# Aster32/GAN-DANet

Measured on AMD Instinct MI355X. Metric: train samples/sec (G+D step) on 256x256 tiles, higher is better.
Workload: dtype bf16; 1 GPU; full G+D train step, 8ch 256x256 -> 1024x1024 tiles, batch 32/GPU (global 32), perceptual=on, SSIM evaluated, AdamW x2; survey_config=3, per_gpu_batch=32, global_batch=32, tile=256, parallelism=dp1

## Files before the change

gan-danet_amd/_lib.py:

```python
from __future__ import annotations

import ctypes as C
import os

HERE = os.path.dirname(os.path.abspath(__file__))
LIB_PATH = os.path.join(HERE, "lib", "libgandanet_hip.so")

PREC_FP32, PREC_BF16, PREC_X3 = 0, 1, 2
PAM_BWD_K64_ATOMIC, PAM_BWD_K64_PARTS, PAM_BWD_K32_PARTS, PAM_BWD_TWO_KERNEL = 0, 1, 2, 3
ACT_NONE, ACT_RELU, ACT_LEAKY02, ACT_SIGMOID = 0, 1, 2, 3
EVAL_F64, EVAL_SKIP_NAN = 1, 2
GUARD_SQNORM, GUARD_NORM, GUARD_COEF, GUARD_OK, GUARD_APPLIED, GUARD_SKIPPED, GUARD_RECORD = range(7)
GUARD_CHUNK = 65536
FILTER_F32, FILTER_F64 = 0, 1
EDGE_REFLECT, EDGE_INTERIOR = 0, 1
FILTER_MAX_RADIUS, SAVGOL_MAX_WINDOW = 64, 33
ZOOM_MIRROR, ZOOM_NEAREST = 0, 1
FREQ_MAX_BINS, FREQ_MAX_TABLE_BYTES = 33, 16 << 20
ZONE_MAX, ZONE_EDGE_CHUNK = 32, 512
STL_MAX_T = 2048

c_fp = C.c_void_p


# ... 151 lines not shown
    "gd_spline_prefilter_axis": (_i, [_p, _p, _i, _l, _l, _l, _p]),
    "gd_restore_units": (_i, [_p, _i, _p, _i, _p, _l, _l, C.c_double, C.c_double, C.c_double, _p, _i, _p]),
    "gd_masked_plane_mean_f64_ws_bytes": (_sz, [_l, _l]),
    "gd_masked_plane_mean_f64": (_i, [_p, _l, _l, _p, _p, _p, _p, _sz, _p]),
    "gd_blend_region": (_i, [_p, _p, _p, _i, _i, _i, _i, _i, _i, _i, _p]),
    "gd_channel_moments_ws_bytes": (_sz, [_l, _l]),
    "gd_channel_moments": (_i, [_p, _i, _l, _l, _p, _p, _sz, _p]),
    "gd_scale_from_moments_host": (_i, [C.POINTER(C.c_double), _l, C.POINTER(C.c_double), C.POINTER(C.c_double),
                                        C.POINTER(C.c_double)]),
    "gd_channel_affine": (_i, [_p, _i, _p, _i, _l, _l, _p, _p, _i, _l, _l, _p]),
    "gd_freq_cos_table_host": (_i, [_l, _i, C.POINTER(C.c_double)]),
    "gd_freq_augment_axis": (_i, [_p, _p, _i, _l, _l, _l, _p, _i, _p, _p]),
    "gd_zone_rasterize": (_i, [_p, _l, C.POINTER(_l), _i, _p, _l, _p, _l, _p, _p]),
    "gd_zone_rasterize_host": (_i, [C.POINTER(C.c_double), _l, C.POINTER(_l), _i, C.POINTER(C.c_double), _l, C.POINTER(C.c_double), _l,
                                    C.POINTER(C.c_uint32)]),
    "gd_zone_mean_ws_bytes": (_sz, [_l, _l, _i]),
    "gd_zone_mean": (_i, [_p, _i, _l, _l, _p, _i, _p, _p, _p, _p, _sz, _p]),
    "gd_stl_decompose": (_i, [_p, _i, _l, _l, _i, _i, _i, _i, _i, _i, _i, _i, _i, _p, _p, _p, _p, _p]),
    "gd_stl_decompose_host": (_i, [_p, _i, _l, _l, _i, _i, _i, _i, _i, _i, _i, _i, _i, _p, _p, _p, _p]),
    "gd_augment_d4": (_i, [_p, _p, _i, _i, _i, _i, _p, _p, _f, _p]),
    "gd_bcast_mul": (_i, [_p, _p, _p, _i, _i, _l, _i, _p]),
    "gd_row_dot": (_i, [_p, _p, _p, _l, _l, _p]),
    "gd_chan_maxmean_fwd": (_i, [_p, _p, _p, _i, _i, _l, _p]),
    "gd_chan_maxmean_bwd": (_i, [_p, _p, _p, _i, _i, _l, _p]),
    "gd_comm_unique_id": (_i, [C.c_char_p]),
    "gd_comm_init": (_i, [_i, _i, C.c_char_p]),
    "gd_comm_world": (_i, []),
    "gd_allreduce": (_i, [_p, _sz, _i, _p]),
    "gd_reduce_scatter": (_i, [_p, _p, _sz, _i, _p]),
    "gd_allgather": (_i, [_p, _p, _sz, _i, _p]),
    "gd_comm_destroy": (_i, []),
    "gd_pack_bf16": (_i, [_p, _l, _i, _i, _i, _p, _f, _p, _i, _i, _p, _i, _i, _i, _i, _p]),
    "gd_pack_16": (_i, [_p, _l, _i, _i, _i, _p, _f, _p, _i, _i, _p, _i, _i, _i, _i, _i, _p]),
    "gd_pack_16_affine": (_i, [_p, _l, _i, _i, _i, _p, _p, _i, _p, _i, _i, _p, _i, _i, _i, _p]),
}

_lib = None


class GandanetError(RuntimeError):
    pass


def load() -> C.CDLL:
    global _lib
    if _lib is not None:
        return _lib
    if not os.path.exists(LIB_PATH):
        raise GandanetError(
            f"{LIB_PATH} is missing: the HIP extension is not built (run __graft_entry__.build()). "
            "There is no CPU fallback.")
    lib = C.CDLL(LIB_PATH)
    for name, (res, args) in SIGNATURES.items():
        fn = getattr(lib, name)
        fn.restype = res
        fn.argtypes = args
    if lib.gd_sizeof_conv_desc() != C.sizeof(ConvDesc) or lib.gd_sizeof_gemm_nt_desc() != C.sizeof(GemmNTDesc):
        raise GandanetError("descriptor struct layout differs between _lib.py and libgandanet_hip.so")
    _lib = lib
    return lib


def last_error() -> str:
    buf = C.create_string_buffer(512)
    load().gd_last_error(buf, 512)
    return buf.value.decode()
# ... 6 lines not shown
```

gan-danet_amd/csrc/gemm_conv.hip:

```cpp
#include <stdlib.h>

#include <type_traits>

#include "common.h"
#include "tile_mma.h"
#include "../../include/gandanet.h"

namespace {

using gd::TILE_BK;
using gd::TILE_BN;
constexpr int BN = TILE_BN;
constexpr int BK = TILE_BK;

template <int BM, int MODE>
__global__ __launch_bounds__(256) void conv_nn_kernel(const gd_conv_desc d) {
    constexpr bool BF16 = MODE != gd::MODE_F32;
    constexpr bool X3 = MODE == gd::MODE_X3;
    using P = gd::TilePol<MODE>;
    using elem = typename P::elem;
    constexpr int LD = P::LD;
    constexpr int WAVES_N = gd::TileGeom<BM>::WAVES_N;
    constexpr int TM = gd::TileGeom<BM>::TM;
    constexpr int TN = gd::TileGeom<BM>::TN;
// ... 450 lines not shown
    const float alpha = d.alpha ? *d.alpha : 1.f;
#pragma unroll
    for (int sb = 0; sb < NS; ++sb)
#pragma unroll
    for (int i = 0; i < TM; ++i)
#pragma unroll
        for (int j = 0; j < TN; ++j) {
            const int pn = n0 + sb * BN + wn * TN * 32 + j * 32 + r;
            if (pn >= HW) continue;
            float rsv[16], oldv[16];
#pragma unroll
            for (int e = 0; e < 16; ++e) {
                const int m = m0 + wm * TM * 32 + i * 32 + gd::acc_row(e, h);
                rsv[e] = (d.res && m < d.M) ? d.res[(long)b * d.res_bs + (long)m * HW + pn] : 0.f;
            }
#pragma unroll
            for (int e = 0; e < 16; ++e) {
                const int m = m0 + wm * TM * 32 + i * 32 + gd::acc_row(e, h);
                oldv[e] = (d.accumulate && m < d.M) ? reinterpret_cast<const float*>(d.y)[(long)b * d.y_bs + (long)m * HW + pn] : 0.f;
            }
#pragma unroll
            for (int e = 0; e < 16; ++e) {
                const int m = m0 + wm * TM * 32 + i * 32 + gd::acc_row(e, h);
                if (m >= d.M) continue;
                float v = acc[sb][i][j][e] * alpha + rsv[e];
                if (d.bias) v += d.bias[m];
                if (d.act == GD_ACT_RELU) v = fmaxf(v, 0.f);
                else if (d.act == GD_ACT_LEAKY02) v = v >= 0.f ? v : 0.2f * v;
                reinterpret_cast<float*>(d.y)[(long)b * d.y_bs + (long)m * HW + pn] = v + oldv[e];
            }
        }
}

template <int BM, bool X3 = false>
__global__ __launch_bounds__(256) void conv1x1_tr_plain_kernel(const gd_conv_desc d) {
    constexpr int LDA = BK + 8;
    constexpr int A_PL = BM * LDA, X_PL = BK * XLD;
    constexpr int WAVES_N = gd::TileGeom<BM>::WAVES_N;
    constexpr int TM = gd::TileGeom<BM>::TM;
    constexpr int TN = gd::TileGeom<BM>::TN;
    constexpr int KPT_A = BM / 8;
    __shared__ __attribute__((aligned(16))) unsigned short As[(X3 ? 2 : 1) * BM * LDA];
    __shared__ __attribute__((aligned(16))) unsigned short Xs[(X3 ? 2 : 1) * BK * XLD];

    const int tid = threadIdx.x, lane = tid & 63, wave = tid >> 6;
    const int r = lane & 31, h = lane >> 5;
    const int wm = wave / WAVES_N, wn = wave % WAVES_N;
    const int b = blockIdx.z, m0 = blockIdx.y * BM, n0 = blockIdx.x * BN;
    const int HW = d.Ho * d.Wo;

    const int am = tid % BM, akg = tid / BM;
    const bool a_row_ok = (m0 + am) < d.M;
    const float* a_row = d.a + (long)b * d.a_bs + (long)(m0 + am) * d.a_sm;

    const int xq = tid & 31, xr0 = tid >> 5;
    const float* x_img = d.x + (long)b * d.x_bs;
    const int pq = n0 + xq * 4;
    const bool q_full = pq + 3 < HW;

    f32x16_t acc[TM][TN];
#pragma unroll
    for (int i = 0; i < TM; ++i)
#pragma unroll
        for (int j = 0; j < TN; ++j)
#pragma unroll
            for (int e = 0; e < 16; ++e) acc[i][j][e] = 0.f;

    float ra[KPT_A];
    float4 rx[4];
    const int T = (d.Ck + BK - 1) / BK;
    auto load_tile = [&](int t) {
        const int c0 = t * BK;
#pragma unroll
        for (int i = 0; i < KPT_A; ++i) {
            const int c = c0 + akg * KPT_A + i;
            ra[i] = (a_row_ok && c < d.Ck) ? a_row[(long)c * d.a_sc] : 0.f;
        }
#pragma unroll
        for (int i = 0; i < 4; ++i) {
            const int c = c0 + xr0 + 8 * i;
            float4 v = make_float4(0.f, 0.f, 0.f, 0.f);
            if (c < d.Ck) {
                const float* p = x_img + (long)c * HW + pq;
                if (q_full) {
                    v = *reinterpret_cast<const float4*>(p);
                } else {
// ... 104 lines not shown
            for (int i = 0; i < TM; ++i)
                fa[i] = *reinterpret_cast<const bf16x8_t*>(As + (wm * TM * 32 + i * 32 + r) * LDA + ks * 16 + 8 * h);
#pragma unroll
            for (int j = 0; j < TN; ++j) {
                const unsigned short* p = Xs + (ks * 16 + 8 * h + tq) * XLD + (wn * TN + j) * 32 + 16 * tg + 4 * tp;
                const s16x4_t lo = __builtin_amdgcn_ds_read_tr16_b64_v4i16((__attribute__((address_space(3))) s16x4_t*)p);
                const s16x4_t hi = __builtin_amdgcn_ds_read_tr16_b64_v4i16(
                    (__attribute__((address_space(3))) s16x4_t*)(p + 4 * XLD));
                fb[j] = bf16x8_t{lo.x, lo.y, lo.z, lo.w, hi.x, hi.y, hi.z, hi.w};
            }
#pragma unroll
            for (int i = 0; i < TM; ++i)
#pragma unroll
                for (int j = 0; j < TN; ++j)
                    acc[i][j] = __builtin_amdgcn_mfma_f32_32x32x16_bf16(
                        __builtin_bit_cast(gd::bf16x8_native_t, fa[i]), __builtin_bit_cast(gd::bf16x8_native_t, fb[j]),
                        acc[i][j], 0, 0, 0);
        }
    };

    load_tile(0);
    store_tile();
    __syncthreads();
    for (int t = 0; t < T; ++t) {
        if (t + 1 < T) load_tile(t + 1);
        compute_tile();
        __syncthreads();
        if (t + 1 < T) {
            store_tile();
            __syncthreads();
        }
    }

    const float alpha = d.alpha ? *d.alpha : 1.f;
#pragma unroll
    for (int i = 0; i < TM; ++i)
#pragma unroll
        for (int j = 0; j < TN; ++j) {
            const int pn = n0 + wn * TN * 32 + j * 32 + r;
            if (pn >= HW) continue;
            float rsv[16], oldv[16];
#pragma unroll
            for (int e = 0; e < 16; ++e) {
                const int m = m0 + wm * TM * 32 + i * 32 + gd::acc_row(e, h);
                rsv[e] = (d.res && m < d.M) ? d.res[(long)b * d.res_bs + (long)m * HW + pn] : 0.f;
            }
#pragma unroll
            for (int e = 0; e < 16; ++e) {
                const int m = m0 + wm * TM * 32 + i * 32 + gd::acc_row(e, h);
                oldv[e] = (d.accumulate && m < d.M) ? reinterpret_cast<const float*>(d.y)[(long)b * d.y_bs + (long)m * HW + pn] : 0.f;
            }
#pragma unroll
            for (int e = 0; e < 16; ++e) {
                const int m = m0 + wm * TM * 32 + i * 32 + gd::acc_row(e, h);
                if (m >= d.M) continue;
                float v = acc[i][j][e] * alpha + rsv[e];
                if (d.bias) v += d.bias[m];
                if (d.act == GD_ACT_RELU) v = fmaxf(v, 0.f);
                else if (d.act == GD_ACT_LEAKY02) v = v >= 0.f ? v : 0.2f * v;
                reinterpret_cast<float*>(d.y)[(long)b * d.y_bs + (long)m * HW + pn] = v + oldv[e];
            }
        }
}

static bool conv1x1_tr_eligible(const gd_conv_desc& d) {
    const long HW = (long)d.Ho * d.Wo;
    return d.ks == 1 && d.stride == 1 && d.pad == 0 && (d.precision == GD_PREC_BF16 || d.precision == GD_PREC_X3) && d.out_layout == 0 && !d.out_bf16 &&
           (d.Mstore == 0 || d.Mstore == d.M) && d.Hi == d.Ho && d.Wi == d.Wo && HW % 4 == 0 && d.x_bs % 4 == 0 &&
           ((uintptr_t)d.x % 16) == 0;
}

template <int BM>
int launch(const gd_conv_desc& d, hipStream_t s) {
    const int sstep = d.sub_step > 1 ? d.sub_step : 1;
    const long hs = (d.Ho - d.sub_oy + sstep - 1) / sstep, ws = (d.Wo - d.sub_ox + sstep - 1) / sstep;
    if (hs <= 0 || ws <= 0) return 0;
    dim3 grid(gd_cdiv(hs * ws, BN), gd_cdiv(d.Mstore, BM), d.B);
    if (d.precision == GD_PREC_BF16)
        hipLaunchKernelGGL((conv_nn_kernel<BM, gd::MODE_BF16>), grid, dim3(256), 0, s, d);
    else if (d.precision == GD_PREC_X3)
        hipLaunchKernelGGL((conv_nn_kernel<BM, gd::MODE_X3>), grid, dim3(256), 0, s, d);
    else
        hipLaunchKernelGGL((conv_nn_kernel<BM, gd::MODE_F32>), grid, dim3(256), 0, s, d);
    GD_LAUNCH_CHECK();
    return 0;
}

}

extern "C" int gd_conv2d(const gd_conv_desc* dp, void* stream) {
    GD_CHECK_ARG(dp != nullptr, "gd_conv2d: null descriptor");
    gd_conv_desc d = *dp;
    if (d.Mstore < d.M) d.Mstore = d.M;
    GD_CHECK_ARG(d.B > 0 && d.M > 0 && d.Ck > 0 && d.ks > 0 && d.stride > 0 && d.pad >= 0, "gd_conv2d: bad sizes");
    GD_CHECK_ARG(d.Hi > 0 && d.Wi > 0 && d.Ho > 0 && d.Wo > 0, "gd_conv2d: bad spatial sizes");
// ... 26 lines not shown
        if (d.precision == GD_PREC_X3) {
            if (bm == 32) hipLaunchKernelGGL((conv1x1_tr_plain_kernel<32, true>), grid, dim3(256), 0, s, d);
            else if (bm == 64) hipLaunchKernelGGL((conv1x1_tr_plain_kernel<64, true>), grid, dim3(256), 0, s, d);
            else hipLaunchKernelGGL((conv1x1_tr_plain_kernel<128, true>), grid, dim3(256), 0, s, d);
        } else if (ns == 1) {
            if (bm == 32) hipLaunchKernelGGL((conv1x1_tr_plain_kernel<32>), grid, dim3(256), 0, s, d);
            else if (bm == 64) hipLaunchKernelGGL((conv1x1_tr_plain_kernel<64>), grid, dim3(256), 0, s, d);
            else hipLaunchKernelGGL((conv1x1_tr_plain_kernel<128>), grid, dim3(256), 0, s, d);
        } else
        if (bm == 32) { if (ns == 4) GD_C1X1(32, 4); else if (ns == 2) GD_C1X1(32, 2); else GD_C1X1(32, 1); }
        else if (bm == 64) { if (ns == 4) GD_C1X1(64, 4); else if (ns == 2) GD_C1X1(64, 2); else GD_C1X1(64, 1); }
        else { if (ns == 2) GD_C1X1(128, 2); else GD_C1X1(128, 1); }
#undef GD_C1X1
        GD_LAUNCH_CHECK();
        return 0;
    }
    auto run = [&](const gd_conv_desc& dd) -> int {
        if (dd.Mstore <= 32) return launch<32>(dd, s);
        if (dd.Mstore <= 64 || (dd.Mstore % 128 != 0 && dd.Mstore % 128 <= 64)) return launch<64>(dd, s);
        return launch<128>(dd, s);
    };
    if (d.transposed && d.stride > 1 && d.sub_step <= 1) {
        for (int py = 0; py < d.stride; ++py)
            for (int px = 0; px < d.stride; ++px) {
                gd_conv_desc dd = d;
                dd.sub_oy = py; dd.sub_ox = px; dd.sub_step = d.stride;
                const int rc = run(dd);
                if (rc) return rc;
            }
        return 0;
    }
    return run(d);
}
```

gan-danet_amd/kern.py:

```python
from __future__ import annotations

import ctypes as C
import math
import os
from typing import Optional, Tuple

import torch

from . import _lib as L

Tensor = torch.Tensor


def _stream() -> int:
    return torch.cuda.current_stream().cuda_stream


def _ptr(t: Optional[Tensor]):
    return None if t is None else t.data_ptr()


def _chk(t: Tensor, name: str = "tensor", dtype=torch.float32) -> None:
    if not t.is_cuda:
        raise L.GandanetError(f"{name}: expected a GPU tensor (there is no CPU fallback in the product path)")
# ... 601 lines not shown
    db = torch.empty_like(b) if need_b else None
    L.check(lib().gd_ssim_bwd(_ptr(a), _ptr(b), _ptr(gscale), B, Cn, H, W, window, _ptr(coef), _ptr(da), _ptr(db),
                              _stream()), "gd_ssim_bwd")
    return da, db


def adamw(p: Tensor, g: Tensor, m: Tensor, v: Tensor, step: int, lr: float, beta1: float, beta2: float, eps: float,
          weight_decay: float, grad_scale: float = 1.0) -> None:
    for t in (p, g, m, v):
        _dense(t, "adamw tensor")
    L.check(lib().gd_adamw(_ptr(p), _ptr(g), _ptr(m), _ptr(v), p.numel(), step, lr, beta1, beta2, eps, weight_decay,
                           grad_scale, _stream()), "gd_adamw")


LOG2E = 1.4426950408889634


def pack_bf16(s: Tensor, R: int, Cc: int, *, scale: Optional[Tensor] = None, scale_imm: float = 1.0, plain_shape=None,
              t_shape=None, perm16: bool = False, ones_row: int = -1, f16: bool = False):
    sbs = _bview(s, "pack input")
    B = s.shape[0]
    plain = tr = None
    rp = ldp = ccp = ldt = 0
    dt = torch.float16 if f16 else torch.bfloat16
    if plain_shape is not None:
        rp, ldp = plain_shape
        plain = torch.empty(B, rp, ldp, device=s.device, dtype=dt)
    if t_shape is not None:
        ccp, ldt = t_shape
        tr = torch.empty(B, ccp, ldt, device=s.device, dtype=dt)
    L.check(lib().gd_pack_16(_ptr(s), sbs, B, R, Cc, _ptr(scale), float(scale_imm), _ptr(plain), rp, ldp, _ptr(tr),
                             ccp, ldt, int(perm16), int(ones_row), int(f16), _stream()), "gd_pack_16")
    return plain, tr


def pack_nhwc16_affine(x: Tensor, scale: Optional[Tensor], shift: Optional[Tensor], relu: bool) -> Tensor:
    sbs = _bview(x, "pack input")
    B, Cn, H, W = x.shape
    out = torch.empty(B, H * W, Cn, device=x.device, dtype=torch.bfloat16)
    L.check(lib().gd_pack_16_affine(_ptr(x), sbs, B, Cn, H * W, _ptr(scale), _ptr(shift), int(relu), None, 0, 0, _ptr(out),
                                    H * W, Cn, 0, _stream()), "gd_pack_16_affine")
    return out


def augment_d4(x: Tensor, ops: Tensor, noise: Optional[Tensor] = None, noise_scale: float = 0.05) -> Tensor:
    _dense(x, "augment input")
    _chk(ops, "augment ops", torch.int32)
    B, Cn, H, W = x.shape
    if ops.numel() != B or (noise is not None and _dense(noise, "noise").shape != x.shape):
        raise L.GandanetError("augment_d4: ops must hold one word per sample and noise must match the batch")
    y = torch.empty_like(x)
    L.check(lib().gd_augment_d4(_ptr(x), _ptr(y), B, Cn, H, W, _ptr(ops), _ptr(noise), float(noise_scale), _stream()),
            "gd_augment_d4")
    return y


def bcast_mul(x: Tensor, att: Tensor, mode: int) -> Tensor:
    _dense(x), _dense(att)
    B, Cn = x.shape[0], x.shape[1]
    HW = x[0, 0].numel()
    if att.numel() != (B * Cn if mode == 0 else B * HW):
        raise L.GandanetError(f"bcast_mul: gate of {att.numel()} elements does not match x {tuple(x.shape)} (mode {mode})")
    y = torch.empty_like(x)
    L.check(lib().gd_bcast_mul(_ptr(x), _ptr(att), _ptr(y), B, Cn, HW, mode, _stream()), "gd_bcast_mul")
    return y

# ... 962 lines not shown
```

gan-danet_amd/ops.py:

```python
from __future__ import annotations

import os
from typing import List, Optional

import torch
from torch.autograd import Function

from . import _lib as L
from . import kern as K
from .config import config, operand_mode, sixteen_bit

ACT_NONE, ACT_RELU, ACT_LEAKY, ACT_SIGMOID = L.ACT_NONE, L.ACT_RELU, L.ACT_LEAKY02, L.ACT_SIGMOID


def _prec(layer: str = "other") -> int:
    mode = operand_mode(layer)
    return L.PREC_BF16 if mode == "16" else L.PREC_X3 if mode == "x3" else L.PREC_FP32


def _x3(layer: str) -> bool:
    return operand_mode(layer) == "x3"


def _x3_eligible(x, w, stride, pad, act) -> bool:
# ... 32 lines not shown
        for w, b in zip(ws[1:], bs[1:]):
            acts.append(K.conv3x3_nhwc_s2(acts[-1], K.conv3x3_operator(_c(w), "fwd", sp), b, w.shape[0], 2, Disc1TrunkFn.SLOPE,
                                          split=sp))
        ctx.save_for_backward(x, *ws, *acts)
        ctx.has_bias = tuple(b is not None for b in bs)
        ctx.split = sp
        return K.nhwc_flatten_fwd(acts[-1], split=sp)

    @staticmethod
    def backward(ctx, df):
        x, *rest = ctx.saved_tensors
        ws, acts = rest[:4], rest[4:]
        need = ctx.needs_input_grad
        sp = ctx.split
        grads = [None] * 9
        g = K.nhwc_flatten_bwd(_c(df), acts[3], Disc1TrunkFn.SLOPE, split=sp)
        for l in (3, 2, 1):
            if need[1 + 2 * l] or need[2 + 2 * l]:
                dw, db = K.conv3x3_wgrad_nhwc(g, acts[l - 1], 2, ctx.has_bias[l] and need[2 + 2 * l], split=sp)
                grads[1 + 2 * l], grads[2 + 2 * l] = (dw if need[1 + 2 * l] else None), db
            g = K.conv3x3_nhwc_s2_dgrad(g, K.conv3x3_operator(_c(ws[l]), "dgrad_s2", sp), acts[l - 1], Disc1TrunkFn.SLOPE,
                                        split=sp)
        if need[1] or need[2]:
            dw, db = K.disc_stem_wgrad(g, x, ctx.has_bias[0] and need[2], split=sp)
            grads[1], grads[2] = (dw if need[1] else None), db
        if need[0]:
            grads[0] = K.disc_stem_dgrad(g, _c(ws[0]), x.shape[2], x.shape[3], split=sp)
        return tuple(grads)


CONV_WIDE_NHWC = os.environ.get("GD_CONV_WIDE_NHWC", "1") != "0"
DENSE_NHWC = os.environ.get("GD_DENSE_NHWC", "1") != "0"
PAM_CAT = os.environ.get("GD_PAM_CAT", "1") != "0"
WIDE_MIN_CIN = int(os.environ.get("GD_WIDE_MIN_CIN", "128"))


def _wide3x3(x, w, stride, pad, act, prec) -> bool:
    return (CONV_WIDE_NHWC and prec == L.PREC_BF16 and x.dim() == 4 and tuple(w.shape[2:]) == (3, 3) and stride == 1
            and pad == 1 and act in (ACT_NONE, ACT_RELU) and w.shape[1] >= WIDE_MIN_CIN and w.shape[1] % 8 == 0 and w.shape[0] > 32
            and w.shape[0] % 8 == 0 and (x.shape[2] * x.shape[3]) % 8 == 0)


def _pack3x3_x(x, split, scale=None, shift=None, relu=False):
    if split:
        return K.pack_split(x, scale=scale, shift=shift, relu=relu)[1]
    if scale is not None:
        return K.pack_nhwc16_affine(x, scale, shift, relu)
    B, Cin, H, W = x.shape
    return K.pack_bf16(x, Cin, H * W, t_shape=(H * W, Cin))[1]


def _packed3x3_fwd(x16, w, bias, H, W, split, relu=False, out=None):
    return K.conv3x3_nhwc_f32out(x16, K.conv3x3_operator(_c(w), "fwd", split), bias, w.shape[0], H, W, relu=relu, out=out)


def _packed3x3_bwd(dy, x16, w, H, W, split, need_dx, need_dw, mask=None, dw_first=False):
    if not (need_dx or need_dw):
        return None, None
    Cout, N = dy.shape[1], H * W
    if split:
        dyp, dyt = K.pack_split(_as3(dy), want_plain=need_dw, want_tr=need_dx, mask=None if mask is None else _as3(mask))
    else:
        dyp, dyt = K.pack_bf16(_as3(dy), Cout, N, plain_shape=(Cout, N) if need_dw else None,
                               t_shape=(N, Cout) if need_dx else None)

    def wgrad():
# ... 244 lines not shown


def _pad_plane(t: torch.Tensor, N: int, Np: int) -> torch.Tensor:
    if N == Np:
        return t
    B, R = t.shape[0], t.shape[1]
    out = torch.zeros(B, R, Np, device=t.device, dtype=torch.float32)
    K.copy_rows(t, K._bview(t), N, out, R * Np, Np, B, R, N)
    return out


def _pam_pack16(q, k, v, r, Cn, N, D, ones_row, f16):
    Np, Cp = _npad(N), _cp(Cn)
    _, qt = K.pack_bf16(q, r, N, scale_imm=K.LOG2E, t_shape=(Np, D), f16=f16)
    kn, kt = K.pack_bf16(k, r, N, plain_shape=(D, Np), t_shape=(Np, D), perm16=True, ones_row=D - 1, f16=f16)
    vn, vt = K.pack_bf16(v, Cn, N, plain_shape=(Cp, Np), t_shape=(Np, Cp), perm16=True, ones_row=ones_row, f16=f16)
    return qt, kt, kn, vn, vt


def _pam_route(B: int, Cn: int, r: int, N: int) -> str:
    if sixteen_bit("pam") and Cn <= 192 and r <= 31:
        return "narrow"
    if _pam_wide(Cn, r):
        return "wide"
    return "f32" if _pam_f32(B, Cn, r, N) else "chain"


def _pam_forward(x, wq, bq, wk, bk, wv, bv, gamma_p, out3, prec):
    B, Cn, H, W = x.shape
    N = H * W
    r = wq.shape[0]
    x3 = x.view(B, Cn, N)
    route = _pam_route(B, Cn, r, N)
    if route != "chain" and PAM_CAT and (bq is None) == (bk is None) == (bv is None):
        wc = torch.empty(2 * r + Cn, Cn, 1, 1, device=x.device, dtype=torch.float32)
        for w_, lo in ((wq, 0), (wk, r), (wv, 2 * r)):
            K.copy_slab(_c(w_).view(1, w_.shape[0], Cn), wc.view(1, 2 * r + Cn, Cn)[:, lo:lo + w_.shape[0]])
        bc = None
        if bq is not None:
            bc = torch.empty(2 * r + Cn, device=x.device, dtype=torch.float32)
            for b_, lo in ((bq, 0), (bk, r), (bv, 2 * r)):
                K.copy_slab(b_.view(1, -1, 1), bc.view(1, -1, 1)[:, lo:lo + b_.numel()])
        y3 = K.conv2d_fwd(x, wc, bc, 1, 0, prec).view(B, 2 * r + Cn, N)
        q, k, v = y3[:, :r], y3[:, r:2 * r], y3[:, 2 * r:]
    else:
        q = K.conv2d_fwd(x, wq, bq, 1, 0, prec).view(B, r, N)
        k = K.conv2d_fwd(x, wk, bk, 1, 0, prec).view(B, r, N)
        v = K.conv2d_fwd(x, wv, bv, 1, 0, prec).view(B, Cn, N)
    if route in ("narrow", "wide"):
        Np, Cp = _npad(N), _cp(Cn)
        f16 = _pam_f16()
        D = 32 if route == "narrow" else K.pam_wide_slots(r)
        ones = Cp - 1 if route == "narrow" and Cn < Cp else -1
        qt, kt, kn, vn, vt = _pam_pack16(q, k, v, r, Cn, N, D, ones, f16)
        del q, k, v
        y3 = None
        o_attn = torch.empty(B, Cn, N, device=x.device, dtype=torch.float32)
        lse = torch.empty(B, N, device=x.device, dtype=torch.float32)
        if route == "wide":
            K.pam_wide_fwd(qt, kt, vn, B, N, Np, Cn, Cp, D, gamma_p, x3, out3, o_attn, lse, r_alg=r, f16=f16)
        elif K.PAM_SHIFT and not f16:
            K.pam_flash_fwd_shift(qt, kt, vn, B, N, Np, Cn, Cp, gamma_p, x3, out3, o_attn, lse, r_alg=r, v_ones=ones >= 0)
        else:
            k_sqmax = K.pam_key_sqnorm_max(kt, N, f16) if K.PAM_NOMAX else None
            K.pam_flash_fwd(qt, kt, vn, B, N, Np, Cn, Cp, gamma_p, x3, out3, o_attn, lse, r_alg=r, v_ones=ones >= 0, f16=f16,
                            k_sqmax=k_sqmax)
        return route, (qt, kt, kn, vt, o_attn, lse)
    if route == "f32":
        Np = _npad(N)
        q, k, v = _pad_plane(q, N, Np), _pad_plane(k, N, Np), _pad_plane(v, N, Np)
        o_attn = torch.empty(B, Cn, N, device=x.device, dtype=torch.float32)
        lse = torch.empty(B, N, device=x.device, dtype=torch.float32)
        K.pam_f32_fwd(q, k, v, B, N, Np, Cn, r, gamma_p, x3, out3, o_attn, lse)
        return route, (q, k, v, o_attn, lse)
    prec = prec if sixteen_bit("pam") else L.PREC_FP32
    return route, _pam_chain_fwd(q, k, v, x3, gamma_p, out3, prec)


def _pam_chain_fwd(q, k, v, x3, gamma_p, out3, prec):
    B, r, N = q.shape
    Cn = v.shape[1]
    qt_, kt_ = K.transpose(q), K.transpose(k)
    s = torch.empty(B, N, N, device=q.device, dtype=torch.float32)
    K.gemm_nt(B=B, M=N, N=N, kseg=1, klen=r, a=qt_, a_bs=N * r, a_ss=0, lda=r, bm=kt_, b_bs=N * r, b_ss=0,
              ldb=r, c=s, c_bs=N * N, ldc=N, precision=prec, splits=1)
    p = K.softmax_rows(s, 1.0, out=s)
    o_attn = torch.empty(B, Cn, N, device=q.device, dtype=torch.float32)
# ... 692 lines not shown
```

include/gandanet.h:

```cpp
#ifndef GANDANET_H
#define GANDANET_H
#include <stddef.h>
#include <stdint.h>
#ifdef __cplusplus
extern "C" {
#endif

#define GD_VERSION 100
void gd_set_deterministic(int on);
int gd_get_deterministic(void);
int gd_set_det_reduce(int mode);
int gd_get_det_reduce(void);
int gd_version(void);
int gd_last_error(char* buf, int n);
int gd_sizeof_conv_desc(void);
int gd_sizeof_gemm_nt_desc(void);

enum { GD_PREC_FP32 = 0,
       GD_PREC_BF16 = 1,
       GD_PREC_X3 = 2     };
enum { GD_ACT_NONE = 0, GD_ACT_RELU = 1, GD_ACT_LEAKY02 = 2, GD_ACT_SIGMOID = 3 };

typedef struct gd_conv_desc {
    int B;
// ... 179 lines not shown
                         float logit_scale, float* received, void* stream);
int gd_pam_attn_rows(const float* q, long q_bs, const float* k, long k_bs, const int* idx, int S, int B, int N, int Npad, int r,
                     float logit_scale, float* rows, float* lse_rows, void* stream);
int gd_round_to_16(const float* x, float* y, long n, float scale, int f16, void* stream);

size_t gd_hist_match_ws_bytes(long ns, long nt);
int gd_hist_match(const float* src, const float* ref, int B, long ns, long nt, double weight, double* out, void* ws,
                  size_t ws_bytes, void* stream);
int gd_blend_region(float* gen, const float* grace, const float* mask, int BC, int H, int W, int sr, int er, int sc,
                    int ec, void* stream);
int gd_augment_d4(const float* src, float* dst, int B, int C, int H, int W, const int* ops, const float* noise,
                  float noise_scale, void* stream);
int gd_bcast_mul(const float* x, const float* att, float* y, int B, int C, long HW, int mode, void* stream);
int gd_row_dot(const float* a, const float* b, float* out, long rows, long n, void* stream);
int gd_chan_maxmean_fwd(const float* x, float* y, int* idx, int B, int C, long HW, void* stream);
int gd_chan_maxmean_bwd(const float* dy, const int* idx, float* dx, int B, int C, long HW, void* stream);
int gd_chan_dot(const float* a, long a_bs, const float* o, long o_bs, int B, int C, int N, const float* gamma,
                float* d_raw, float* delta, void* stream);
int gd_pack_16_split(const float* s, long s_bs, int B, int R, int Cc, const float* row_scale, const float* row_shift, int relu,
                     void* plain, long p_bs, int ldp, long p_cs, int p_ncopy, int p_pattern, void* tr, long t_bs, int ldt,
                     long t_cs, int t_ncopy, int t_pattern, void* stream);
int gd_pack_16_split_masked(const float* s, long s_bs, int B, int R, int Cc, const float* row_scale, const float* row_shift,
                            int relu, void* plain, long p_bs, int ldp, long p_cs, int p_ncopy, int p_pattern, void* tr, long t_bs,
                            int ldt, long t_cs, int t_ncopy, int t_pattern, const float* mask, long m_bs, void* stream);
int gd_split3_weights(const float* w, long A, long Bn, long Cn, float* out, void* stream);
int gd_pam_f16_scale(const float* dout, long dout_bs, int B, int C, int N, const float* gamma, float* delta, float* scales,
                     float* ws, void* stream);
int gd_pack_bf16(const float* s, long s_bs, int B, int R, int Cc, const float* scale_dev, float scale_imm, void* plain,
                 int Rp_plain, int ld_plain, void* transposed, int Ccp_t, int ld_t, int perm16, int ones_row,
                 void* stream);
int gd_pack_16(const float* s, long s_bs, int B, int R, int Cc, const float* scale_dev, float scale_imm, void* plain,
               int Rp_plain, int ld_plain, void* transposed, int Ccp_t, int ld_t, int perm16, int ones_row, int f16,
               void* stream);
int gd_pack_16_affine(const float* s, long s_bs, int B, int R, int Cc, const float* row_scale, const float* row_shift, int relu,
                      void* plain, int Rp_plain, int ld_plain, void* transposed, int Ccp_t, int ld_t, int f16, void* stream);

int gd_comm_unique_id(char* id128);
int gd_comm_init(int rank, int world, const char* id128);
int gd_comm_world(void);
int gd_allreduce(void* buf, size_t n, int dtype, void* stream);
int gd_reduce_scatter(const void* send, void* recv, size_t recv_n, int dtype, void* stream);
int gd_allgather(const void* send, void* recv, size_t send_n, int dtype, void* stream);
int gd_comm_destroy(void);

enum { GD_EVAL_F64 = 1, GD_EVAL_SKIP_NAN = 2 };
size_t gd_eval_stats_ws_bytes(long n);
int gd_eval_stats(const void* pred, const void* truth, long planes, long hw, const unsigned char* mask, double a, double b,
                  int flags, double* rec, void* ws, size_t ws_bytes, void* stream);
size_t gd_masked_plane_mean_ws_bytes(long planes, long hw);
int gd_masked_plane_mean(const float* x, long planes, long hw, const unsigned char* mask, double* mean, long long* count,
                         void* ws, size_t ws_bytes, void* stream);
int gd_ensemble_stats(const void* x, int M, long member_stride, long n, int f64, void* mean, void* std_out, void* stream);
int gd_eval_merge_host(const double* recs, long k, double* rec_out, double* metrics);

enum { GD_GUARD_SQNORM = 0, GD_GUARD_NORM = 1, GD_GUARD_COEF = 2, GD_GUARD_OK = 3, GD_GUARD_APPLIED = 4, GD_GUARD_SKIPPED = 5,
       GD_GUARD_RECORD = 6 };
#define GD_GUARD_CHUNK 65536L
size_t gd_grad_sqnorm_ws_bytes(long total_chunks);
int gd_grad_sqnorm(const float* const* grads, const long* ns, int count, float gscale, int accumulate, double* rec, void* ws,
                   size_t ws_bytes, void* stream);
int gd_guard_finalize(double* rec, double max_norm, int skip_nonfinite, void* stream);
int gd_adamw_guarded(float* p, const float* g, float* m, float* v, float* ema, long n, const double* rec, float lr, float beta1,
                     float beta2, float eps, float weight_decay, float grad_scale, float ema_decay, void* stream);

enum { GD_FILTER_F32 = 0, GD_FILTER_F64 = 1 };
enum { GD_EDGE_REFLECT = 0, GD_EDGE_INTERIOR = 1 };
// ... 58 lines not shown
```

Baseline: 37.92 samples/s.

## Fuse PAM q/k/v 1x1 projections with 16-bit attention operand packing

Measured after the change: 38.06 samples/s (median of 6 runs). About the same (+0.4%).

```diff
diff --git a/gan-danet_amd/_lib.py b/gan-danet_amd/_lib.py
--- a/gan-danet_amd/_lib.py
+++ b/gan-danet_amd/_lib.py
@@ -207,6 +207,8 @@
     "gd_comm_destroy": (_i, []),
     "gd_pack_bf16": (_i, [_p, _l, _i, _i, _i, _p, _f, _p, _i, _i, _p, _i, _i, _i, _i, _p]),
     "gd_pack_16": (_i, [_p, _l, _i, _i, _i, _p, _f, _p, _i, _i, _p, _i, _i, _i, _i, _i, _p]),
+    "gd_pam_proj_pack_eligible": (_i, [_p, _l, _i, _i, _i, _i, _i, _p, _p, _p, _p, _p, _p, _i, _i, _i, _i, _i, _p, _p, _p, _p, _p]),
+    "gd_pam_proj_pack": (_i, [_p, _l, _i, _i, _i, _i, _i, _p, _p, _p, _p, _p, _p, _i, _i, _i, _i, _i, _i, _f, _p, _p, _p, _p, _p, _p]),
     "gd_pack_16_affine": (_i, [_p, _l, _i, _i, _i, _p, _p, _i, _p, _i, _i, _p, _i, _i, _i, _p]),
 }
 
diff --git a/gan-danet_amd/csrc/gemm_conv.hip b/gan-danet_amd/csrc/gemm_conv.hip
--- a/gan-danet_amd/csrc/gemm_conv.hip
+++ b/gan-danet_amd/csrc/gemm_conv.hip
@@ -506,8 +506,16 @@
         }
 }
 
-template <int BM, bool X3 = false>
-__global__ __launch_bounds__(256) void conv1x1_tr_plain_kernel(const gd_conv_desc d) {
+struct PamPackArgs {
+    const float *wq, *wk, *wv;
+    const float *bq, *bk, *bv;
+    unsigned short *qt, *kt, *kn, *vn, *vt;
+    int r, C, D, Cp, Np, ones_row, f16;
+    float qscale;
+};
+
+template <int BM, bool X3, bool PACK>
+__device__ __forceinline__ void conv1x1_tr_plain_body(const gd_conv_desc d, const PamPackArgs pk) {
     constexpr int LDA = BK + 8;
     constexpr int A_PL = BM * LDA, X_PL = BK * XLD;
     constexpr int WAVES_N = gd::TileGeom<BM>::WAVES_N;
@@ -524,8 +532,10 @@
     const int HW = d.Ho * d.Wo;
 
     const int am = tid % BM, akg = tid / BM;
-    const bool a_row_ok = (m0 + am) < d.M;
-    const float* a_row = d.a + (long)b * d.a_bs + (long)(m0 + am) * d.a_sm;
+    const int a_seg = (m0 + am) < pk.D ? 0 : (m0 + am) < 2 * pk.D ? 1 : 2, a_rr = m0 + am - a_seg * pk.D;
+    const bool a_row_ok = PACK ? a_rr < (a_seg == 2 ? pk.C : pk.r) : (m0 + am) < d.M;
+    const float* a_row = PACK ? (a_seg == 0 ? pk.wq : a_seg == 1 ? pk.wk : pk.wv) + (long)a_rr * d.Ck
+                              : d.a + (long)b * d.a_bs + (long)(m0 + am) * d.a_sm;
 
     const int xq = tid & 31, xr0 = tid >> 5;
     const float* x_img = d.x + (long)b * d.x_bs;
@@ -696,6 +706,78 @@
         }
     }
 
+    if constexpr (PACK) {
+        constexpr int SLD = 40;
+        static_assert(4 * 32 * SLD <= BM * LDA, "per-wave scratch must fit the A image");
+        unsigned short* st = As + wave * 32 * SLD;
+        const PamPackArgs& a = pk;
+        const int f16 = a.f16;
+        auto cvt2 = [f16](float lo, float hi) -> unsigned int {
+            if (f16) {
+                const unsigned int l = __builtin_bit_cast(unsigned short, (_Float16)lo), u = __builtin_bit_cast(unsigned short, (_Float16)hi);
+                return l | (u << 16);
+            }
+            return gd_pack_bf2(lo, hi);
+        };
+#pragma unroll
+        for (int i = 0; i < TM; ++i) {
+            const int R0 = m0 + wm * TM * 32 + i * 32;
+            if (R0 >= d.M) continue;
+            const int seg = R0 < a.D ? 0 : R0 < 2 * a.D ? 1 : 2;
+            const int s0 = R0 - seg * a.D;
+            const int real = seg == 2 ? a.C : a.r;
+            const int ones = seg == 0 ? -1 : seg == 1 ? a.D - 1 : a.ones_row;
+            const float* bias = seg == 0 ? a.bq : seg == 1 ? a.bk : a.bv;
+            const float k = seg == 0 ? a.qscale : 1.f;
+            const int ldt = seg == 2 ? a.Cp : a.D;
+            unsigned short* tr = (seg == 0 ? a.qt : seg == 1 ? a.kt : a.vt) + (long)b * a.Np * ldt;
+            unsigned short* pl = seg == 0 ? nullptr : (seg == 1 ? a.kn : a.vn) + (long)b * ldt * a.Np;
+#pragma unroll
+            for (int j = 0; j < TN; ++j) {
+                const int P0 = n0 + wn * TN * 32 + j * 32;
+                const bool px_ok = P0 + r < HW;
+#pragma unroll
+                for (int g = 0; g < 4; ++g) {
+                    float v[4];
+#pragma unroll
+                    for (int t = 0; t < 4; ++t) {
+                        const int ch = s0 + 8 * g + 4 * h + t;
+                        float x = acc[i][j][4 * g + t];
+                        if (bias && ch < real) x += bias[ch];
+                        x = fmaf(x, k, 0.f);
+                        v[t] = ch == ones ? 1.f : (ch < real && px_ok) ? x : 0.f;
+                    }
+                    uint2 w;
+                    w.x = cvt2(v[0], v[1]);
+                    w.y = cvt2(v[2], v[3]);
+                    *reinterpret_cast<uint2*>(st + r * SLD + 8 * g + 4 * h) = w;
+                }
+                __builtin_amdgcn_wave_barrier();
+#pragma unroll
+                for (int kk = 0; kk < 2; ++kk) {
+                    const int sidx = lane + 64 * kk, px = sidx >> 2, sg = sidx & 3;
+                    const uint4 o = *reinterpret_cast<const uint4*>(st + px * SLD + 8 * sg);
+                    *reinterpret_cast<uint4*>(tr + (long)(P0 + px) * ldt + s0 + 8 * sg) = o;
+                }
+                if (pl) {
+#pragma unroll
+                    for (int kk = 0; kk < 2; ++kk) {
+                        const int sidx = lane + 64 * kk, ch = sidx & 31, pg = sidx >> 5;
+                        const int base = 16 * (pg >> 1) + 4 * (pg & 1);
+                        unsigned int w[4];
+#pragma unroll
+                        for (int t = 0; t < 2; ++t) {
+                            w[t] = (unsigned int)st[(base + 2 * t) * SLD + ch] | ((unsigned int)st[(base + 2 * t + 1) * SLD + ch] << 16);
+                            w[2 + t] = (unsigned int)st[(base + 8 + 2 * t) * SLD + ch] | ((unsigned int)st[(base + 9 + 2 * t) * SLD + ch] << 16);
+                        }
+                        *reinterpret_cast<uint4*>(pl + (long)(s0 + ch) * a.Np + P0 + 8 * pg) = make_uint4(w[0], w[1], w[2], w[3]);
+                    }
+                }
+                __builtin_amdgcn_wave_barrier();
+            }
+        }
+        return;
+    }
     const float alpha = d.alpha ? *d.alpha : 1.f;
 #pragma unroll
     for (int i = 0; i < TM; ++i)
@@ -725,6 +807,15 @@
                 reinterpret_cast<float*>(d.y)[(long)b * d.y_bs + (long)m * HW + pn] = v + oldv[e];
             }
         }
+}
+
+template <int BM, bool X3 = false>
+__global__ __launch_bounds__(256) void conv1x1_tr_plain_kernel(const gd_conv_desc d) {
+    conv1x1_tr_plain_body<BM, X3, false>(d, PamPackArgs{});
+}
+template <bool X3>
+__global__ __launch_bounds__(256) void pam_proj_pack_kernel(const gd_conv_desc d, const PamPackArgs pk) {
+    conv1x1_tr_plain_body<128, X3, true>(d, pk);
 }
 
 static bool conv1x1_tr_eligible(const gd_conv_desc& d) {
@@ -817,3 +908,49 @@
     }
     return run(d);
 }
+
+static const char* pam_proj_pack_reason(const float* x, long x_bs, int B, int C, int r, int H, int W, const float* wq, const float* wk,
+                                        const float* wv, const float* bq, const float* bk, const float* bv, int D, int Np, int Cp,
+                                        int ones_row, int precision, const void* qt, const void* kt, const void* kn, const void* vn,
+                                        const void* vt) {
+    if (!(x && wq && wk && wv && qt && kt && kn && vn && vt)) return "gd_pam_proj_pack: null tensor";
+    if (!(B > 0 && B <= 65535 && C > 0 && r > 0 && H > 0 && W > 0)) return "gd_pam_proj_pack: bad sizes";
+    if ((bq == nullptr) != (bk == nullptr) || (bq == nullptr) != (bv == nullptr)) return "gd_pam_proj_pack: unsupported: q / k / v biases must be all present or all absent";
+    if (precision != GD_PREC_BF16 && precision != GD_PREC_X3) return "gd_pam_proj_pack: unsupported precision (bf16 or split-bf16 products only)";
+    if ((D != 32 && D != 64) || r > D - 1) return "gd_pam_proj_pack: unsupported: D must be 32 or 64 with r <= D - 1";
+    if (Cp != (C + 31) / 32 * 32) return "gd_pam_proj_pack: Cp must be C rounded up to 32";
+    const long HW = (long)H * W;
+    if (HW >= (1L << 31) - 256 || Np % 128 != 0 || Np < HW) return "gd_pam_proj_pack: Np must be a multiple of 128, >= H * W";
+    if (ones_row != -1 && (ones_row < C || ones_row >= Cp)) return "gd_pam_proj_pack: ones_row must be a padding row of V";
+    if (HW % 4 != 0 || x_bs % 4 != 0 || ((uintptr_t)x % 16) != 0) return "gd_pam_proj_pack: unsupported: needs H * W % 4 == 0 and 16-byte aligned images";
+    if (((uintptr_t)qt | (uintptr_t)kt | (uintptr_t)kn | (uintptr_t)vn | (uintptr_t)vt) % 16 != 0) return "gd_pam_proj_pack: operands must be 16-byte aligned";
+    static const int tr_env = getenv("GD_CONV1X1_TR") ? atoi(getenv("GD_CONV1X1_TR")) : 1;
+    if (!tr_env) return "gd_pam_proj_pack: unsupported: the transposed-read 1x1 kernels are switched off (GD_CONV1X1_TR=0)";
+    return nullptr;
+}
+extern "C" int gd_pam_proj_pack_eligible(const float* x, long x_bs, int B, int C, int r, int H, int W, const float* wq, const float* wk,
+                                         const float* wv, const float* bq, const float* bk, const float* bv, int D, int Np, int Cp,
+                                         int ones_row, int precision, const void* qt, const void* kt, const void* kn, const void* vn,
+                                         const void* vt) {
+    return pam_proj_pack_reason(x, x_bs, B, C, r, H, W, wq, wk, wv, bq, bk, bv, D, Np, Cp, ones_row, precision, qt, kt, kn, vn, vt) == nullptr;
+}
+extern "C" int gd_pam_proj_pack(const float* x, long x_bs, int B, int C, int r, int H, int W, const float* wq, const float* wk,
+                                const float* wv, const float* bq, const float* bk, const float* bv, int D, int Np, int Cp, int ones_row,
+                                int precision, int f16, float q_scale, void* qt, void* kt, void* kn, void* vn, void* vt, void* stream) {
+    const char* why = pam_proj_pack_reason(x, x_bs, B, C, r, H, W, wq, wk, wv, bq, bk, bv, D, Np, Cp, ones_row, precision, qt, kt, kn, vn, vt);
+    GD_CHECK_ARG(why == nullptr, why);
+    gd_conv_desc d = {};
+    d.B = B; d.M = d.Mstore = 2 * D + Cp; d.Ck = C; d.ks = 1; d.stride = 1;
+    d.Hi = d.Ho = H; d.Wi = d.Wo = W;
+    d.a = wq; d.a_sm = C; d.a_sc = 1; d.a_st = 1;
+    d.x = x; d.x_bs = x_bs;
+    d.precision = precision;
+    PamPackArgs pk = {wq, wk, wv, bq, bk, bv, (unsigned short*)qt, (unsigned short*)kt, (unsigned short*)kn, (unsigned short*)vn,
+                      (unsigned short*)vt, r, C, D, Cp, Np, ones_row, f16 ? 1 : 0, q_scale};
+    dim3 grid(Np / BN, gd_cdiv(d.M, 128), B);
+    hipStream_t s = (hipStream_t)stream;
+    if (precision == GD_PREC_X3) hipLaunchKernelGGL((pam_proj_pack_kernel<true>), grid, dim3(256), 0, s, d, pk);
+    else hipLaunchKernelGGL((pam_proj_pack_kernel<false>), grid, dim3(256), 0, s, d, pk);
+    GD_LAUNCH_CHECK();
+    return 0;
+}
diff --git a/gan-danet_amd/kern.py b/gan-danet_amd/kern.py
--- a/gan-danet_amd/kern.py
+++ b/gan-danet_amd/kern.py
@@ -657,6 +657,33 @@
     L.check(lib().gd_pack_16(_ptr(s), sbs, B, R, Cc, _ptr(scale), float(scale_imm), _ptr(plain), rp, ldp, _ptr(tr),
                              ccp, ldt, int(perm16), int(ones_row), int(f16), _stream()), "gd_pack_16")
     return plain, tr
+
+
+def pam_proj_pack(x: Tensor, wq: Tensor, bq: Optional[Tensor], wk: Tensor, bk: Optional[Tensor], wv: Tensor,
+                  bv: Optional[Tensor], D: int, Np: int, Cp: int, ones_row: int, precision: int, f16: bool):
+    xbs = _bview(x, "projection input")
+    B, Cn, H, W = x.shape
+    r = wq.shape[0]
+    for t in (wq, wk, wv):
+        _dense(t, "projection weight")
+    for t in (bq, bk, bv):
+        if t is not None:
+            _dense(t, "projection bias")
+    if tuple(wq.shape) != (r, Cn, 1, 1) or tuple(wk.shape) != (r, Cn, 1, 1) or tuple(wv.shape) != (Cn, Cn, 1, 1):
+        raise L.GandanetError("pam_proj_pack: weight shapes do not match the input")
+    dt = torch.float16 if f16 else torch.bfloat16
+    qt = torch.empty(B, Np, D, device=x.device, dtype=dt)
+    kt = torch.empty(B, Np, D, device=x.device, dtype=dt)
+    kn = torch.empty(B, D, Np, device=x.device, dtype=dt)
+    vn = torch.empty(B, Cp, Np, device=x.device, dtype=dt)
+    vt = torch.empty(B, Np, Cp, device=x.device, dtype=dt)
+    head = (_ptr(x), xbs, B, Cn, r, H, W, _ptr(wq), _ptr(wk), _ptr(wv), _ptr(bq), _ptr(bk), _ptr(bv), D, Np, Cp, int(ones_row),
+            precision)
+    outs = (_ptr(qt), _ptr(kt), _ptr(kn), _ptr(vn), _ptr(vt))
+    if not lib().gd_pam_proj_pack_eligible(*head, *outs):
+        return None
+    L.check(lib().gd_pam_proj_pack(*head, int(f16), float(LOG2E), *outs, _stream()), "gd_pam_proj_pack")
+    return qt, kt, kn, vn, vt
 
 
 def pack_nhwc16_affine(x: Tensor, scale: Optional[Tensor], shift: Optional[Tensor], relu: bool) -> Tensor:
diff --git a/gan-danet_amd/ops.py b/gan-danet_amd/ops.py
--- a/gan-danet_amd/ops.py
+++ b/gan-danet_amd/ops.py
@@ -88,6 +88,7 @@
 CONV_WIDE_NHWC = os.environ.get("GD_CONV_WIDE_NHWC", "1") != "0"
 DENSE_NHWC = os.environ.get("GD_DENSE_NHWC", "1") != "0"
 PAM_CAT = os.environ.get("GD_PAM_CAT", "1") != "0"
+PAM_PROJ_PACK = os.environ.get("GD_PAM_PROJ_PACK", "1") != "0"
 WIDE_MIN_CIN = int(os.environ.get("GD_WIDE_MIN_CIN", "128"))
 
 
@@ -398,7 +399,14 @@
     r = wq.shape[0]
     x3 = x.view(B, Cn, N)
     route = _pam_route(B, Cn, r, N)
-    if route != "chain" and PAM_CAT and (bq is None) == (bk is None) == (bv is None):
+    packed = None
+    if route in ("narrow", "wide") and PAM_PROJ_PACK and (bq is None) == (bk is None) == (bv is None):
+        D = 32 if route == "narrow" else K.pam_wide_slots(r)
+        ones = _cp(Cn) - 1 if route == "narrow" and Cn < _cp(Cn) else -1
+        packed = K.pam_proj_pack(x, _c(wq), bq, _c(wk), bk, _c(wv), bv, D, _npad(N), _cp(Cn), ones, prec, _pam_f16())
+    if packed is not None:
+        q = k = v = None
+    elif route != "chain" and PAM_CAT and (bq is None) == (bk is None) == (bv is None):
         wc = torch.empty(2 * r + Cn, Cn, 1, 1, device=x.device, dtype=torch.float32)
         for w_, lo in ((wq, 0), (wk, r), (wv, 2 * r)):
             K.copy_slab(_c(w_).view(1, w_.shape[0], Cn), wc.view(1, 2 * r + Cn, Cn)[:, lo:lo + w_.shape[0]])
@@ -418,7 +426,10 @@
         f16 = _pam_f16()
         D = 32 if route == "narrow" else K.pam_wide_slots(r)
         ones = Cp - 1 if route == "narrow" and Cn < Cp else -1
-        qt, kt, kn, vn, vt = _pam_pack16(q, k, v, r, Cn, N, D, ones, f16)
+        if packed is not None:
+            qt, kt, kn, vn, vt = packed
+        else:
+            qt, kt, kn, vn, vt = _pam_pack16(q, k, v, r, Cn, N, D, ones, f16)
         del q, k, v
         y3 = None
         o_attn = torch.empty(B, Cn, N, device=x.device, dtype=torch.float32)
diff --git a/include/gandanet.h b/include/gandanet.h
--- a/include/gandanet.h
+++ b/include/gandanet.h
@@ -235,6 +235,13 @@
 int gd_pack_16(const float* s, long s_bs, int B, int R, int Cc, const float* scale_dev, float scale_imm, void* plain,
                int Rp_plain, int ld_plain, void* transposed, int Ccp_t, int ld_t, int perm16, int ones_row, int f16,
                void* stream);
+int gd_pam_proj_pack_eligible(const float* x, long x_bs, int B, int C, int r, int H, int W, const float* wq, const float* wk,
+                              const float* wv, const float* bq, const float* bk, const float* bv, int D, int Np, int Cp,
+                              int ones_row, int precision, const void* qt, const void* kt, const void* kn, const void* vn,
+                              const void* vt);
+int gd_pam_proj_pack(const float* x, long x_bs, int B, int C, int r, int H, int W, const float* wq, const float* wk,
+                     const float* wv, const float* bq, const float* bk, const float* bv, int D, int Np, int Cp, int ones_row,
+                     int precision, int f16, float q_scale, void* qt, void* kt, void* kn, void* vn, void* vt, void* stream);
 int gd_pack_16_affine(const float* s, long s_bs, int B, int R, int Cc, const float* row_scale, const float* row_shift, int relu,
                       void* plain, int Rp_plain, int ld_plain, void* transposed, int Ccp_t, int ld_t, int f16, void* stream);
 
```
